# VUmcCGP/wisecondor

Hardware: NVIDIA B200
Metric: newref_bin_pairs_per_s (higher is better)
Workload: dtype f64

## Files before the change

wisecondor_b200/csrc/wc_common.cuh:

```cuda
#pragma once
#include <cuda.h>
#include <cuda_runtime.h>
#include <stdint.h>
#include <stdio.h>
#include <string.h>
#include <math.h>
#include <string>
#include <vector>
#include <algorithm>
#include "../../include/wisecondor_b200.h"

void wc_set_error(const char* fmt, ...);

#define WC_CUDA(expr)                                                                                   \
    do {                                                                                                \
        cudaError_t _e = (expr);                                                                        \
        if (_e != cudaSuccess) {                                                                        \
            wc_set_error("%s failed: %s (%s:%d)", #expr, cudaGetErrorString(_e), __FILE__, __LINE__);   \
            return WC_ERR_CUDA;                                                                         \
        }                                                                                               \
    } while (0)

#define WC_CHECK_ARG(cond)                                                                              \
    do {                                                                                                \
// ... 7 lines not shown
    void* p = nullptr;
    size_t bytes = 0;
};

enum { WC_NBUF = 56, WC_NPHASE = 12, WC_NCOUNTER = 12 };

enum {
    SLOT_XC = 0, SLOT_NORMS, SLOT_ROWCS, SLOT_ROWCE, SLOT_RBMETA, SLOT_CAND_D, SLOT_CAND_J, SLOT_SEGCNT,
    SLOT_SEGFLAG, SLOT_SLOW, SLOT_SCRATCH, SLOT_IO_X, SLOT_IO_IDX, SLOT_IO_DIST, SLOT_ROWTHR,
    SLOT_IN_KEY, SLOT_IN_J, SLOT_IN_CNT, SLOT_N32, SLOT_F16STAT,
    SLOT_PROF = 20, SLOT_PIV_IDS = 21, SLOT_PIV_X = 22, SLOT_PIV_N = 23, SLOT_PIV_META = 37, SLOT_S_STACK = 38,
    SLOT_T_COPY = 24, SLOT_T_ZT, SLOT_T_RT, SLOT_T_NT, SLOT_T_SD, SLOT_T_FLAGS, SLOT_T_TOTALS, SLOT_T_PROJ,
    SLOT_T_REVCNT = 44, SLOT_T_REVCUR, SLOT_T_DIRTY, SLOT_T_PAIRS,
    SLOT_S_ZC = 32, SLOT_S_META, SLOT_S_STATUS, SLOT_S_RC, SLOT_S_AUX,
    SLOT_P_FIRST = 40,
    SLOT_FIN_J = 48, SLOT_FIN_D, SLOT_FIN_P, SLOT_FIN_GRP
};

struct wc_shard_plan {
    int valid = 0;
    int N = 0, S = 0, k = 0, cap = 0, in_cap = 0, world = 1, rank = 0;
    int nb = 0, bp = 0, b0 = 0, b1 = 0;
    int row0 = 0, row1 = 0, rows_per = 0;
    int nkc = 0, nd_last = 0, extra_h = 0, ld = 0, nstages = 0, nrb = 0, nseg = 0, gridA = 0, gridB = 0;
    size_t Npad = 0, smem = 0, nlistA = 0;
    long long tilesA = 0, tilesB = 0, tiles_plain = 0;
    double mcoef = 0.0, madd = 0.0;
    int f16 = 0, ldh = 0;
    int pivots = 0;
    const double* corrected = nullptr;
    const unsigned long long* thr = nullptr;
// ... 125 lines not shown
```

wisecondor_b200/csrc/wc_search.cu:

```cuda
#include "wc_common.cuh"
#include <cuda_fp16.h>

namespace {

typedef unsigned long long u64;

constexpr int BM = 128;
constexpr int BN = 128;
constexpr int BK = 16;
constexpr int CONSUMER_WARPS = 8;
constexpr int CONSUMER_THREADS = CONSUMER_WARPS * 32;
constexpr int WROWS = BM / CONSUMER_WARPS;
constexpr int PRODUCER_WARPS = 4;
constexpr int TOPK_THREADS = CONSUMER_THREADS + PRODUCER_WARPS * 32;
constexpr int TILE_BYTES = BM * BK * 8;
constexpr int STAGE_BYTES = 2 * TILE_BYTES;
constexpr int MAX_STAGES = 6;
constexpr int HIST_BINS = 256;
constexpr int FIN_THREADS = 128;
constexpr int FIN_CHUNK = 32;
constexpr int FIN_BUCKETS = 1024;
constexpr int FIN_ECAP = 1360;
constexpr int EXH_THREADS = 256;
constexpr int STG = 128;
// ... 92 lines not shown
}
__device__ __forceinline__ int bucket_of(double d, double mn, float scale) {
    int b = (int)((float)(d - mn) * scale);
    return b < 0 ? 0 : (b > HIST_BINS - 1 ? HIST_BINS - 1 : b);
}
__device__ __forceinline__ u64 key_of_tau(double tau) { return (u64)__double_as_longlong(-0.5 * tau); }
inline u64 host_key_of_tau(double tau) {
    const double v = -0.5 * tau;
    u64 bits;
    memcpy(&bits, &v, sizeof(bits));
    return bits;
}
__device__ __forceinline__ double dist_of_key(u64 key) { return -2.0 * __longlong_as_double((long long)key); }
template <typename Args>
__device__ __forceinline__ double madd_of(const Args& a) { return a.madd_p != nullptr ? __ldg(a.madd_p) : a.madd; }

template <int PER_LANE>
__device__ __noinline__ void prune_row(u64* ck, int* cj, int n, int k, double nrm, double mcoef, double madd, int lane,
                                       u64* sk, int* sj, u64* thr_out, int* n_out) {
    (void)sk; (void)sj;
    u64 d[PER_LANE];
    int j[PER_LANE];
#pragma unroll
    for (int t = 0; t < PER_LANE; ++t) {
        const int i = t * 32 + lane;
        d[t] = i < n ? __ldcg(ck + i) : ~0ull;
        j[t] = i < n ? __ldcg(cj + i) : 0;
    }
    u64 lo = ~0ull, hi = 0ull;
#pragma unroll
// ... 477 lines not shown
    int k;
    int shortcap;
    double mcoef;
    int* idx_out;
    double* dist_out;
    int* slow_list;
    int* slow_count;
    int slow_bias;
    int vec;
    const u64* in_key;
    const int* in_j;
    const int* in_cnt;
    int in_cap;
    double madd;
    const double* madd_p;
    const u64* row_thr;
    int in_nsrc;
    int in_src_rows;
    int* sl_j;
    u64* sl_k;
    int* sl_p;
    int* grp;
    int* grp_count;
    const int* row_list;
    const int* row_count;
    int* stats;
    int* sl_b;
    int* bkt_hist;
    int bkt_shift;
};

template <int FT, bool SPLIT>
__device__ __forceinline__ void finalize_row(const FinArgs& a, const int rloc, unsigned char* fin_raw) {
    constexpr int ecap = FIN_ECAP;
    double* ex_d = reinterpret_cast<double*>(fin_raw + (size_t)ecap * 12);
    int* ex_j = reinterpret_cast<int*>(ex_d + a.shortcap);
    int* hist = ex_j + a.shortcap;
    __shared__ double s_red[2][FT / 32];
    __shared__ int s_total, s_flag, s_p, s_bstar, s_valid;

    const int tid = threadIdx.x, lane = tid & 31, warp = tid >> 5;
    const int row = a.row_begin + rloc;
    const int rb = rloc / BM, rl = rloc % BM;
    const int seg0 = a.rb_seg_first[rb], nseg = a.rb_seg_count[rb];
    int* out_i = a.idx_out + (size_t)rloc * a.k;
// ... 790 lines not shown
            if (sym)
                WC_CUDA(cudaMemcpyAsync(d_sym, sym_tab.data(), sym_tab.size() * sizeof(int), cudaMemcpyHostToDevice, stream));
            ctx->sched_hash = h;
        }
    }
    WC_CUDA(cudaMemsetAsync(slow, 0, sizeof(int), stream));
    WC_CUDA(cudaMemsetAsync(seg_cnt, 0, (size_t)std::max(nseg, 1) * BM * sizeof(int), stream));
    WC_CUDA(cudaMemsetAsync(seg_flag, 0, (size_t)std::max(nseg, 1) * BM * sizeof(int), stream));
    if (sym) WC_CUDA(cudaMemsetAsync(in_cnt, 0, (size_t)rows * sizeof(int), stream));

    bool f16 = ctx->k5_f16 != 0;
    const bool tc = ctx->k5_f16 == 2;
    const int ldh = tc ? (S + 4 + BKH - 1) / BKH * BKH : (S + BKH - 1) / BKH * BKH;
    const int ldx = tc ? ldh + BKH : ldh;
    float* n32 = nullptr;
    double nmax = 0.0;
    const double eps16 = ldexp(1.0, -10) * (1.0 + ldexp(1.0, -11)) + (tc ? 2.0 : 1.0) * (double)ldh * ldexp(1.0, -23) +
                         (tc ? ldexp(1.0, -20) : ldexp(1.0, -21));
    const unsigned long long* f16_stats_d = nullptr;
    WC_CUDA(cudaEventRecord(ctx->ev[0], stream));
    if (f16) {
        unsigned long long* stats;
        if ((rc = wc_reserve(ctx, SLOT_N32, Npad * sizeof(float), (void**)&n32))) return rc;
        if ((rc = wc_reserve(ctx, SLOT_F16STAT, 4 * sizeof(unsigned long long), (void**)&stats))) return rc;
        WC_CUDA(cudaMemsetAsync(stats, 0, 2 * sizeof(unsigned long long), stream));
        wc_prepare_f16_kernel<<<(int)((Npad * 32 + 255) / 256), 256, 0, stream>>>(corrected_d, N, (int)Npad, S, ldh, ldx, tc ? 1 : 0,
                                                                                  reinterpret_cast<__half*>(Xc), norms, n32, stats);
        WC_CUDA(cudaGetLastError());
        if (ctx->k5_f16_checked != 0) {
            f16_stats_d = stats;
            wc_f16_margin_kernel<<<1, 1, 0, stream>>>(stats, S, eps16, reinterpret_cast<double*>(stats + 2));
        } else {
            unsigned long long st_h[2] = {0, 0};
            WC_CUDA(cudaMemcpyAsync(st_h, stats, sizeof(st_h), cudaMemcpyDeviceToHost, stream));
            WC_CUDA(cudaStreamSynchronize(stream));
            memcpy(&nmax, &st_h[0], sizeof(double));
            if (st_h[1] != 0) f16 = false;
        }
    }
    if (!f16) {
        const int blocks = (int)((Npad * 32 + 255) / 256);
        wc_prepare_kernel<<<blocks, 256, 0, stream>>>(corrected_d, N, (int)Npad, S, ld, Sx, Xc, norms);
// ... 113 lines not shown
        ta.cta_piece_begin = d_cta_piece + (gridA + 1);
        launch(true, gridB);
    }
    WC_CUDA(cudaGetLastError());
    WC_CUDA(cudaEventRecord(ctx->ev[3], stream));

    FinArgs fa;
    fa.X = corrected_d; fa.N = N; fa.S = S; fa.norms = norms; fa.row_cs = d_row_cs; fa.row_ce = d_row_ce;
    fa.row_begin = row_begin; fa.row_end = row_end; fa.rb_seg_first = d_seg_first; fa.rb_seg_count = d_seg_count;
    fa.cand_key = cand_key; fa.cand_j = cand_j; fa.seg_cnt = seg_cnt; fa.seg_flag = seg_flag; fa.cap = cap; fa.k = k;
    fa.shortcap = k <= (f16 ? 96 : 128) ? 256 : 512;
    fa.mcoef = filt_mcoef; fa.idx_out = idx_d; fa.dist_out = dist_d; fa.slow_list = slow + 1; fa.slow_count = slow;
    fa.vec = (S % 4 == 0 && (reinterpret_cast<uintptr_t>(corrected_d) & 31) == 0) ? 4 : 1;
    fa.in_key = in_key; fa.in_j = in_j; fa.in_cnt = in_cnt; fa.in_cap = in_cap; fa.in_nsrc = 1; fa.in_src_rows = 0;
    fa.madd = filt_madd; fa.row_thr = row_thr; fa.madd_p = ta.madd_p;
    fa.slow_bias = 0;
    WC_CUDA(cudaEventRecord(ctx->ev[4], stream));
    long long fin_launches = 0;
    const int nparts = (ctx->d2h_idx_h != nullptr && rows >= 16 * BM) ? std::max(1, ctx->k6_parts) : 1;
    ctx->d2h_rows_done = 0;
    for (int pi = 0, r0 = 0; pi < nparts; ++pi) {
        const int r1 = pi + 1 == nparts ? (int)rows : (int)((long long)rows * (pi + 1) / nparts) / BM * BM;
        if (r1 <= r0) continue;
        FinArgs f = fa;
        const int hb = r0 / BM;
        f.row_begin = row_begin + r0; f.row_end = row_begin + r1;
        f.rb_seg_first += hb; f.rb_seg_count += hb;
        f.idx_out += (size_t)r0 * k; f.dist_out += (size_t)r0 * k;
        f.slow_bias = r0;
        if (f.row_thr != nullptr) f.row_thr += r0;
// ... 175 lines not shown
```

wisecondor_b200/csrc/wc_search_f16.cuh:

```cuda
#pragma once

constexpr int BKH = 64;
constexpr int F16_SCRATCH = 4096;

__device__ __forceinline__ void ldsm_x4(uint32_t addr, uint32_t& r0, uint32_t& r1, uint32_t& r2, uint32_t& r3) {
    asm volatile("ldmatrix.sync.aligned.m8n8.x4.shared.b16 {%0,%1,%2,%3}, [%4];"
                 : "=r"(r0), "=r"(r1), "=r"(r2), "=r"(r3) : "r"(addr));
}
__device__ __forceinline__ void hmma_16816(float (&c)[4], uint32_t a0, uint32_t a1, uint32_t a2, uint32_t a3, uint32_t b0,
                                           uint32_t b1) {
    asm volatile("mma.sync.aligned.m16n8k16.row.col.f32.f16.f16.f32 {%0,%1,%2,%3}, {%4,%5,%6,%7}, {%8,%9}, {%0,%1,%2,%3};"
                 : "+f"(c[0]), "+f"(c[1]), "+f"(c[2]), "+f"(c[3]) : "r"(a0), "r"(a1), "r"(a2), "r"(a3), "r"(b0), "r"(b1));
}
__device__ __forceinline__ float tau32_of_key(u64 key) { return __double2float_ru(dist_of_key(key)); }

__global__ void wc_prepare_f16_kernel(const double* __restrict__ X, int N, int Npad, int S, int ldh, int ldx, int fold,
                                      __half* __restrict__ Xh, double* __restrict__ norms, float* __restrict__ n32,
                                      unsigned long long* __restrict__ stats) {
    const int row = (int)(((size_t)blockIdx.x * blockDim.x + threadIdx.x) >> 5);
    const int lane = threadIdx.x & 31;
    if (row >= Npad) return;
    __half* dst = Xh + (size_t)row * ldx;
    double acc = 0.0;
    bool big = false;
    if (row < N) {
        const double* src = X + (size_t)row * S;
        for (int s = lane; s < ldh; s += 32) {
            const double v = s < S ? src[s] - 1.0 : 0.0;
            const __half hv = __double2half(v);
            dst[s] = hv;
            if (fold && s >= ldh - BKH) dst[s + BKH] = hv;
            acc = fma(v, v, acc);
            if (fabs(v) > 60000.0 && fabs(v) < INFINITY) big = true;
        }
    } else {
        for (int s = lane; s < ldx; s += 32) dst[s] = __float2half(0.0f);
    }
#pragma unroll
    for (int o = 16; o > 0; o >>= 1) acc += __shfl_xor_sync(0xffffffffu, acc, o);
    big = __any_sync(0xffffffffu, big);
    __syncwarp();
    if (lane == 0) {
        norms[row] = row < N ? acc : 0.0;
        n32[row] = row < N ? (float)acc : INFINITY;
        if (fold && row < N) {
            const double nh = -0.5 * acc;
            if (!(acc * 0.5 <= 60000.0)) big = true;
            const __half h = __double2half(nh);
            const __half l = __double2half(nh - (double)__half2float(h));
            const __half one = __float2half(1.0f);
            dst[ldh - 4] = h;   dst[ldh - 3] = l;   dst[ldh - 2] = one; dst[ldh - 1] = one;
            dst[ldx - 4] = one; dst[ldx - 3] = one; dst[ldx - 2] = h;   dst[ldx - 1] = l;
        }
        if (row < N && acc < INFINITY) atomicMax(stats, (unsigned long long)__double_as_longlong(acc));
        if (big) atomicOr(stats + 1, 1ull);
    }
}

template <bool SYM>
// ... 348 lines not shown
```

wisecondor_b200/csrc/wc_search_fin.cuh:

```cuda
#pragma once

constexpr int SEL_WARPS = 4;
constexpr int SEL_ECAP = 1024;
constexpr int SEL_EPL = SEL_ECAP / 32;
constexpr int SEL_U = 4;
constexpr int SEL_MAXSRC = 255;
constexpr size_t SEL_WARP_BYTES = (size_t)SEL_ECAP * 12 + (SEL_MAXSRC + 1) * 4 + 12;
constexpr size_t SEL_WARP_STRIDE = (SEL_WARP_BYTES + 15) / 16 * 16;

__global__ void __launch_bounds__(SEL_WARPS * 32) wc_fin_select_kernel(const FinArgs a, int* __restrict__ big_list,
                                                                       int* __restrict__ big_count, int* __restrict__ stats) {
    extern __shared__ __align__(16) unsigned char sel_raw[];
    const int lane = threadIdx.x & 31, warp = threadIdx.x >> 5;
    const int rloc = blockIdx.x * SEL_WARPS + warp;
    const int rows = a.row_end - a.row_begin;
    if (rloc >= rows) return;
    u64* en_k = reinterpret_cast<u64*>(sel_raw + (size_t)warp * SEL_WARP_STRIDE);
    int* en_j = reinterpret_cast<int*>(en_k + SEL_ECAP);
    int* pre = en_j + SEL_ECAP;
    const int row = a.row_begin + rloc;
    const int rb = rloc / BM, rl = rloc % BM;
    const int seg0 = a.rb_seg_first[rb], nseg = a.rb_seg_count[rb];
    const int nsrc = nseg + (a.in_key != nullptr ? a.in_nsrc : 0);
    int* out_i = a.idx_out + (size_t)rloc * a.k;
// ... 78 lines not shown
            if (keep && pos < SEL_ECAP) {
                en_k[pos] = key[u];
                en_j[pos] = jj[u];
            }
            kept += __popc(bm);
        }
    }
    if (kept > SEL_ECAP) { to_big(); return; }
    if (kept == 0) {
        for (int e = lane; e < a.k; e += 32) { out_i[e] = -1; out_d[e] = 1e10; }
        if (lane == 0) a.sl_p[rloc] = -1;
        return;
    }
    __syncwarp();
    u64 d[SEL_EPL];
#pragma unroll
    for (int t = 0; t < SEL_EPL; ++t) d[t] = t * 32 + lane < kept ? en_k[t * 32 + lane] : ~0ull;
    u64 lo = ~0ull, hi = 0ull;
#pragma unroll
    for (int t = 0; t < SEL_EPL; ++t) {
        if (t * 32 + lane < kept) {
            lo = d[t] < lo ? d[t] : lo;
            hi = d[t] > hi ? d[t] : hi;
        }
    }
    lo = warp_min_u64(lo);
    hi = warp_max_u64(hi);
    u64 blo = lo, bhi = hi, cut = hi;
    int c_hi = kept;
    for (int it = 0; it < 70 && c_hi > a.k; ++it) {
        if (bhi - blo < 2) break;
        const u64 mid = blo + ((bhi - blo) >> 1);
// ... 1 lines not shown
#pragma unroll
        for (int t = 0; t < SEL_EPL; ++t) c += d[t] <= mid ? 1 : 0;
#pragma unroll
        for (int o = 16; o > 0; o >>= 1) c += __shfl_xor_sync(0xffffffffu, c, o);
        if (c >= a.k) { bhi = mid; c_hi = c; cut = mid; } else { blo = mid; }
    }
    u64 vstar = 0ull;
#pragma unroll
    for (int t = 0; t < SEL_EPL; ++t)
        if (d[t] <= cut && d[t] > vstar) vstar = d[t];
    vstar = warp_max_u64(vstar);
    const double dv = dist_of_key(vstar);
    double window = fmax(dv, 0.0) + a.mcoef * (a.norms[row] + fabs(dv)) + madd_of(a);
    if (!(window > 1e-300)) window = 1e-300;
    const u64 wkey = key_of_tau(window);
    int p = 0, jmin = 0x7fffffff;
#pragma unroll
    for (int t = 0; t < SEL_EPL; ++t) {
        const bool keep = t * 32 + lane < kept && d[t] <= wkey;
        const unsigned bm = __ballot_sync(0xffffffffu, keep);
        const int pos = p + __popc(bm & ((1u << lane) - 1u));
        if (keep && pos < a.shortcap) {
            const int j = en_j[t * 32 + lane];
            a.sl_j[(size_t)rloc * a.shortcap + pos] = j;
            jmin = min(jmin, j);
        }
        p += __popc(bm);
    }
#pragma unroll
    for (int o = 16; o > 0; o >>= 1) jmin = min(jmin, __shfl_xor_sync(0xffffffffu, jmin, o));
    if (lane == 0) {
        if (p > a.shortcap) {
            a.slow_list[atomicAdd(a.slow_count, 1)] = rloc + a.slow_bias;
            a.sl_p[rloc] = -1;
        } else {
            a.sl_p[rloc] = p;
            const int bkt = min(jmin >> a.bkt_shift, FIN_BUCKETS - 1);
            a.sl_b[rloc] = bkt;
            atomicAdd(a.bkt_hist + bkt, (p + 31) >> 5);
            if (stats != nullptr) { atomicAdd(stats, kept); atomicAdd(stats + 1, p); atomicMax(stats + 2, kept); }
        }
    }
}

constexpr int SELH_WARPS = 8;
constexpr int SELH_BINS = 1024;

__global__ void __launch_bounds__(SELH_WARPS * 32, 5) wc_fin_select_hist_kernel(const FinArgs a, int* __restrict__ big_list,
                                                                            int* __restrict__ big_count, int* __restrict__ stats) {
    __shared__ int s_hist[SELH_WARPS][SELH_BINS];
    __shared__ int s_pre[SELH_WARPS][SEL_MAXSRC + 1];
    const int lane = threadIdx.x & 31, warp = threadIdx.x >> 5;
    const int rloc = blockIdx.x * SELH_WARPS + warp;
    const int rows = a.row_end - a.row_begin;
    if (rloc >= rows) return;
    int* hist = s_hist[warp];
    int* pre = s_pre[warp];
    const int row = a.row_begin + rloc;
    const int rb = rloc / BM, rl = rloc % BM;
    const int seg0 = a.rb_seg_first[rb], nseg = a.rb_seg_count[rb];
    const int nsrc = nseg + (a.in_key != nullptr ? a.in_nsrc : 0);
    int* out_i = a.idx_out + (size_t)rloc * a.k;
// ... 27 lines not shown
        if (s0 == 0 && lane == 0) pre[0] = 0;
        __syncwarp();
    }
    if (__any_sync(0xffffffffu, flagged != 0)) {
        if (lane == 0) { a.slow_list[atomicAdd(a.slow_count, 1)] = rloc + a.slow_bias; a.sl_p[rloc] = -1; }
        return;
    }
    const u64 tfinal = a.row_thr != nullptr ? __ldcg(a.row_thr + rloc) : ~0ull;
    auto sweep = [&](auto&& f) {
        int s = 0, e0 = 0, ns = nsrc > 0 ? pre[1] : 0;
        bool more = true;
        while (more) {
            u64 key[SEL_U];
            int jj[SEL_U];
            bool ok[SEL_U];
#pragma unroll
            for (int u = 0; u < SEL_U; ++u) {
                while (s < nsrc && e0 >= ns) { ++s; e0 = 0; ns = s < nsrc ? pre[s + 1] - pre[s] : 0; }
                key[u] = ~0ull;
                jj[u] = 0;
                ok[u] = false;
                if (s < nsrc) {
                    const int e = e0 + lane;
                    if (e < ns) {
                        ok[u] = true;
                        if (s < nseg) {
                            const size_t off = ((size_t)(seg0 + s) * BM + rl) * a.cap + e;
                            key[u] = a.cand_key[off];
                            jj[u] = a.cand_j[off];
                        } else {
                            const size_t off = ((size_t)(s - nseg) * a.in_src_rows + rloc) * a.in_cap + e;
                            key[u] = a.in_key[off];
                            jj[u] = a.in_j[off];
                        }
                    }
                    e0 += 32;
                } else {
                    more = false;
                }
            }
#pragma unroll
            for (int u = 0; u < SEL_U; ++u) f(key[u], jj[u], ok[u]);
        }
    };
    double d0 = 0.0, dmax = dist_of_key(tfinal);
    if (!(dmax < 1e10)) {
        const double cut = 1e10 + a.mcoef * (a.norms[row] + 1e10) + madd_of(a);
        double mn = INFINITY, mx = -INFINITY;
        sweep([&](u64 key, int, bool valid) {
            const double d = dist_of_key(key);
            if (valid && key <= tfinal && d <= cut) { mn = fmin(mn, d); mx = fmax(mx, d); }
        });
#pragma unroll
        for (int o = 16; o > 0; o >>= 1) {
            mn = fmin(mn, __shfl_xor_sync(0xffffffffu, mn, o));
            mx = fmax(mx, __shfl_xor_sync(0xffffffffu, mx, o));
        }
        if (mx >= mn) { d0 = mn; dmax = mx; } else { dmax = 0.0; }
    }
    const float scale = dmax - d0 > 1e-5 * fabs(dmax) ? (float)SELH_BINS / (float)(dmax - d0) : 0.0f;
    auto bucket = [&](double d) -> int {
        const float x = (float)(d - d0) * scale;
        return x < (float)SELH_BINS ? (x >= 0.0f ? (int)x : 0) : SELH_BINS - 1;
    };
    int kept = 0;
    sweep([&](u64 key, int, bool valid) {
        const bool live = valid && key <= tfinal;
        if (live) atomicAdd(&hist[bucket(dist_of_key(key))], 1);
        kept += __popc(__ballot_sync(0xffffffffu, live));
    });
    if (kept == 0) {
        for (int e = lane; e < a.k; e += 32) { out_i[e] = -1; out_d[e] = 1e10; }
        if (lane == 0) a.sl_p[rloc] = -1;
        return;
    }
    __syncwarp();
    auto kth_bucket = [&](int kk, int& below) -> int {
        constexpr int PER = SELH_BINS / 32;
        static_assert(PER % 32 == 0, "one bank per lane in the rotated read");
        int sum = 0;
#pragma unroll 8
        for (int t = 0; t < PER; ++t) sum += hist[lane * PER + ((t + lane) & (PER - 1))];
        int incl = sum;
// ... 16 lines not shown
                if (lane >= o) inc2 += w;
            }
            const unsigned m2 = __ballot_sync(0xffffffffu, base + inc2 >= kk);
            if (m2) {
                const int l2 = __ffs(m2) - 1;
                below = base + __shfl_sync(0xffffffffu, inc2 - v, l2);
                return lstar * PER + r * 32 + l2;
            }
            base += __shfl_sync(0xffffffffu, inc2, 31);
        }
        return -1;
    };
    int below = 0;
    int bstar = kth_bucket(a.k, below);
    const bool refine = bstar >= 0 && bstar < SELH_BINS - 1 && scale > 0.0f;
    double vstar = dmax;
    if (refine) vstar = fmin(dmax, d0 + (double)(__fdividef((float)(bstar + 1), scale) * (1.0f + 8.0f * 1.1920929e-7f)));
    auto window_key = [&](double v) -> u64 {
        double window = fmax(v, 0.0) + a.mcoef * (a.norms[row] + fabs(v)) + madd_of(a);
        if (!(window > 1e-300)) window = 1e-300;
        const u64 wk = key_of_tau(window);
        return wk > tfinal ? tfinal : wk;
    };
    const u64 wkey = window_key(vstar);
    const int edge_cnt = refine ? hist[bucket(dist_of_key(wkey))] : 0;
    __syncwarp();
    for (int bb = lane; bb < SELH_BINS; bb += 32) hist[bb] = 0;
    __syncwarp();
    const double dscale = (double)scale;
    u64* my_k = a.sl_k + (size_t)rloc * a.shortcap;
    int* my_j = a.sl_j + (size_t)rloc * a.shortcap;
    int p = 0, jmin = 0x7fffffff;
    sweep([&](u64 key, int j, bool valid) {
        const bool keep = valid && key <= wkey;
        const unsigned bm = __ballot_sync(0xffffffffu, keep);
        const int pos = p + __popc(bm & ((1u << lane) - 1u));
        if (keep && pos < a.shortcap) {
            my_j[pos] = j;
            my_k[pos] = key;
            jmin = min(jmin, j);
        }
        p += __popc(bm);
        if (refine && keep) {
            const double d = dist_of_key(key);
            if (bucket(d) == bstar) {
                const double f = ((d - d0) * dscale - (double)bstar) * (double)SELH_BINS;
                atomicAdd(&hist[f < (double)SELH_BINS ? (f >= 0.0 ? (int)f : 0) : SELH_BINS - 1], 1);
            }
        }
    });
    if (p > a.shortcap) {
        if (lane == 0) {
            a.slow_list[atomicAdd(a.slow_count, 1)] = rloc + a.slow_bias;
            a.sl_p[rloc] = -1;
        }
        return;
    }
    __syncwarp();
    if (refine && p > a.k && ((p - 1) >> 5) != ((max(a.k, p - 2 * edge_cnt - 2) - 1) >> 5)) {
        int below2 = 0;
        const int sstar = kth_bucket(a.k - below, below2);
        if (sstar >= 0 && sstar < SELH_BINS - 1) {
            const double v2 = d0 + ((double)bstar + ((double)(sstar + 1) + 1e-3) / (double)SELH_BINS) / dscale;
            const u64 wkey2 = window_key(fmin(vstar, v2));
            if (wkey2 < wkey) {
                int q = 0;
                jmin = 0x7fffffff;
                for (int e0 = 0; e0 < p; e0 += 32) {
                    const int e = e0 + lane;
                    const bool keep = e < p && __ldcg(my_k + e) <= wkey2;
                    const int j = e < p ? __ldcg(my_j + e) : 0;
                    __syncwarp();
                    const unsigned bm = __ballot_sync(0xffffffffu, keep);
                    if (keep) {
                        my_j[q + __popc(bm & ((1u << lane) - 1u))] = j;
                        jmin = min(jmin, j);
                    }
                    q += __popc(bm);
                }
                p = q;
            }
        }
    }
#pragma unroll
    for (int o = 16; o > 0; o >>= 1) jmin = min(jmin, __shfl_xor_sync(0xffffffffu, jmin, o));
// ... 350 lines not shown
    fa.sl_k = reinterpret_cast<u64*>(sl_d);
    if ((rc = wc_reserve(ctx, SLOT_FIN_P, (2 * (size_t)rows + 8 + FIN_BUCKETS) * sizeof(int), (void**)&fa.sl_p))) return rc;
    if ((rc = wc_reserve(ctx, SLOT_FIN_GRP, (size_t)rows * (gpr + 1) * sizeof(int), (void**)&fa.grp))) return rc;
    fa.grp_count = fa.sl_p + rows;
    int* big_count = fa.sl_p + rows + 1;
    int* stats = fa.sl_p + rows + 2;
    fa.sl_b = fa.sl_p + rows + 8;
    fa.bkt_hist = fa.sl_b + rows;
    fa.bkt_shift = 0;
    while (((fa.N - 1) >> fa.bkt_shift) >= FIN_BUCKETS) ++fa.bkt_shift;
    WC_CUDA(cudaMemsetAsync(fa.bkt_hist, 0, FIN_BUCKETS * sizeof(int), stream));
    int* big_list = fa.grp + (size_t)rows * gpr;
    WC_CUDA(cudaMemsetAsync(fa.grp_count, 0, 5 * sizeof(int), stream));
    fa.row_list = nullptr; fa.row_count = nullptr; fa.stats = stats;
    if (ctx->k6_select != 0) {
        wc_fin_select_hist_kernel<<<(rows + SELH_WARPS - 1) / SELH_WARPS, SELH_WARPS * 32, 0, stream>>>(fa, big_list, big_count, stats);
    } else {
        const size_t sel_smem = SEL_WARPS * SEL_WARP_STRIDE;
        WC_CUDA(cudaFuncSetAttribute(wc_fin_select_kernel, cudaFuncAttributeMaxDynamicSharedMemorySize, (int)sel_smem));
        wc_fin_select_kernel<<<(rows + SEL_WARPS - 1) / SEL_WARPS, SEL_WARPS * 32, sel_smem, stream>>>(fa, big_list, big_count, stats);
    }
    WC_CUDA(cudaGetLastError());
    {
        fa.row_list = big_list; fa.row_count = big_count;
        const int g = std::min(rows, 8 * ctx->sm_count);
        if (wide) {
            WC_CUDA(cudaFuncSetAttribute(wc_finalize_kernel<160, true>, cudaFuncAttributeMaxDynamicSharedMemorySize, (int)fin_smem));
            wc_finalize_kernel<160, true><<<g, 160, fin_smem, stream>>>(fa);
        } else {
            WC_CUDA(cudaFuncSetAttribute(wc_finalize_kernel<FIN_THREADS, true>, cudaFuncAttributeMaxDynamicSharedMemorySize, (int)fin_smem));
            wc_finalize_kernel<FIN_THREADS, true><<<g, FIN_THREADS, fin_smem, stream>>>(fa);
        }
        WC_CUDA(cudaGetLastError());
    }
    wc_fin_bucket_scan_kernel<<<1, FIN_BUCKETS, 0, stream>>>(fa.bkt_hist, fa.grp_count);
// ... 76 lines not shown
```

wisecondor_b200/csrc/wc_search_shard.cuh:

```cuda
#pragma once

namespace {

struct ShardDims { int nb, bp, b0, b1, row0, row1, rows_per, in_cap, frac; size_t thr_len; };

ShardDims shard_dims(const wc_ctx* ctx, int N, int k, int world, int rank) {
    ShardDims d;
    d.frac = (ctx != nullptr && ctx->k5_sym >= 2) ? ctx->k5_sym : 8;
    d.nb = (N + BM - 1) / BM;
    d.bp = (d.nb + world - 1) / world;
    d.b0 = std::min(d.nb, rank * d.bp);
    d.b1 = std::min(d.nb, d.b0 + d.bp);
    d.row0 = std::min(N, d.b0 * BM);
    d.row1 = std::min(N, d.b1 * BM);
    d.rows_per = d.bp * BM;
    d.thr_len = (size_t)world * d.rows_per + BN;
    const int want = world == 1 ? 2 * k * d.frac : (4 * k * d.frac + world - 1) / world;
    d.in_cap = 256;
    while (d.in_cap < want) d.in_cap *= 2;
    return d;
}

int shard_launch_pass(wc_ctx* ctx, int pass, unsigned long long* thr_d, unsigned long long* in_key_d, int* in_j_d,
                      int* in_cnt_d, cudaStream_t stream, const std::vector<int>* seg_first = nullptr, int pivots = 0) {
// ... 207 lines not shown
    if ((rc = wc_reserve(ctx, SLOT_SEGFLAG, (size_t)std::max(nseg, 1) * BM * sizeof(int), (void**)&seg_flag))) return rc;
    const int rows = d.row1 - d.row0;
    if ((rc = wc_reserve(ctx, SLOT_SLOW, ((size_t)std::max(rows, 0) + 1) * sizeof(int), (void**)&slow))) return rc;
    WC_CUDA(cudaMemcpyAsync(d_row_cs, row_cs.data(), (size_t)N * sizeof(int), cudaMemcpyHostToDevice, stream));
    WC_CUDA(cudaMemcpyAsync(d_row_ce, row_ce.data(), (size_t)N * sizeof(int), cudaMemcpyHostToDevice, stream));
    WC_CUDA(cudaMemcpyAsync(d_meta, meta.data(), meta.size() * sizeof(int), cudaMemcpyHostToDevice, stream));
    WC_CUDA(cudaMemsetAsync(slow, 0, sizeof(int), stream));
    WC_CUDA(cudaMemsetAsync(seg_cnt, 0, (size_t)std::max(nseg, 1) * BM * sizeof(int), stream));
    WC_CUDA(cudaMemsetAsync(seg_flag, 0, (size_t)std::max(nseg, 1) * BM * sizeof(int), stream));

    bool f16 = ctx->k5_f16 != 0;
    const bool tcf = ctx->k5_f16 == 2;
    const int ldh = tcf ? (S + 4 + BKH - 1) / BKH * BKH : (S + BKH - 1) / BKH * BKH;
    const int ldx = tcf ? ldh + BKH : ldh;
    double nmax = 0.0;
    WC_CUDA(cudaEventRecord(ctx->ev[0], stream));
    if (f16) {
        float* n32;
        unsigned long long* stats;
        if ((rc = wc_reserve(ctx, SLOT_N32, Npad * sizeof(float), (void**)&n32))) return rc;
        if ((rc = wc_reserve(ctx, SLOT_F16STAT, 2 * sizeof(unsigned long long), (void**)&stats))) return rc;
        WC_CUDA(cudaMemsetAsync(stats, 0, 2 * sizeof(unsigned long long), stream));
        wc_prepare_f16_kernel<<<(int)((Npad * 32 + 255) / 256), 256, 0, stream>>>(corrected_d, N, (int)Npad, S, ldh, ldx, tcf ? 1 : 0,
                                                                                  reinterpret_cast<__half*>(Xc), norms, n32, stats);
        WC_CUDA(cudaGetLastError());
        unsigned long long st_h[2] = {0, 0};
        WC_CUDA(cudaMemcpyAsync(st_h, stats, sizeof(st_h), cudaMemcpyDeviceToHost, stream));
        WC_CUDA(cudaStreamSynchronize(stream));
        memcpy(&nmax, &st_h[0], sizeof(double));
        if (st_h[1] != 0) f16 = false;
    }
    if (!f16)
        wc_prepare_kernel<<<(int)((Npad * 32 + 255) / 256), 256, 0, stream>>>(corrected_d, N, (int)Npad, S, ld, Sx, Xc, norms);
    WC_CUDA(cudaGetLastError());
    WC_CUDA(cudaEventRecord(ctx->ev[1], stream));
    const double eps16 = ldexp(1.0, -10) * (1.0 + ldexp(1.0, -11)) + (tcf ? 2.0 : 1.0) * (double)ldh * ldexp(1.0, -23) +
                         (tcf ? ldexp(1.0, -20) : ldexp(1.0, -21));
    const double tau_init = f16 ? 3e38 : 1e10 * (1.0 + 1e-6);
    wc_fill_u64_kernel<<<(unsigned)((N + 255) / 256), 256, 0, stream>>>(thr_d, (size_t)N, host_key_of_tau(tau_init));
    wc_fill_u64_kernel<<<(unsigned)((d.thr_len - N + 255) / 256), 256, 0, stream>>>(thr_d + N, d.thr_len - (size_t)N, KEY_NEVER);
    WC_CUDA(cudaGetLastError());

    pl.N = N; pl.S = S; pl.k = k; pl.cap = cap; pl.in_cap = d.in_cap; pl.world = world; pl.rank = rank;
    pl.nb = nb; pl.bp = d.bp; pl.b0 = d.b0; pl.b1 = d.b1; pl.row0 = d.row0; pl.row1 = d.row1; pl.rows_per = d.rows_per;
    pl.nkc = nkc; pl.nd_last = nd_last; pl.extra_h = nd_last; pl.ld = ld; pl.nrb = nrb; pl.nseg = npieces;
    pl.gridA = gridA; pl.gridB = gridB; pl.Npad = Npad; pl.nlistA = listA.size();
    pl.tilesA = tilesA; pl.tilesB = tilesB; pl.tiles_plain = tiles_plain;
    pl.f16 = f16 ? ctx->k5_f16 : 0;
    pl.ldh = ldh;
    pl.mcoef = f16 ? 2.0 * eps16 : 16.0 * (double)(S + 16) * 1.1102230246251565e-16;
    pl.madd = f16 ? 2.0 * eps16 * nmax + ldexp(1.0, -20) * sqrt((double)S * nmax) : 0.0;
    if (f16) pl.nkc = ldh / BKH;
// ... 59 lines not shown
    if (rows > 0) {
        WC_CHECK_ARG(idx_d != nullptr && dist_d != nullptr);
        const int nrb1 = std::max(pl.nrb, 1);
        FinArgs fa;
        fa.X = pl.corrected; fa.N = pl.N; fa.S = pl.S; fa.norms = static_cast<double*>(ctx->buf[SLOT_NORMS].p);
        fa.row_cs = d_row_cs; fa.row_ce = d_row_ce; fa.row_begin = pl.row0; fa.row_end = pl.row1;
        fa.rb_seg_first = d_meta + 2 * nrb1; fa.rb_seg_count = d_meta + 3 * nrb1;
        fa.cand_key = static_cast<u64*>(ctx->buf[SLOT_CAND_D].p); fa.cand_j = static_cast<int*>(ctx->buf[SLOT_CAND_J].p);
        fa.seg_cnt = static_cast<int*>(ctx->buf[SLOT_SEGCNT].p); fa.seg_flag = static_cast<int*>(ctx->buf[SLOT_SEGFLAG].p);
        fa.cap = pl.cap; fa.k = pl.k; fa.shortcap = pl.k <= (pl.f16 ? 96 : 128) ? 256 : 512; fa.mcoef = pl.mcoef;
        fa.idx_out = idx_d; fa.dist_out = dist_d; fa.slow_list = slow + 1; fa.slow_count = slow; fa.slow_bias = 0;
        fa.vec = (pl.S % 4 == 0 && (reinterpret_cast<uintptr_t>(pl.corrected) & 31) == 0) ? 4 : 1;
        fa.in_key = recv_key_d; fa.in_j = recv_j_d; fa.in_cnt = recv_cnt_d; fa.in_cap = pl.in_cap;
        fa.in_nsrc = pl.world; fa.in_src_rows = pl.rows_per; fa.madd = pl.madd; fa.madd_p = nullptr;
        fa.row_thr = pl.thr != nullptr ? pl.thr + pl.row0 : nullptr;
        WC_CUDA(cudaEventRecord(ctx->ev[4], stream));
        long long fin_launches = 0;
        int rcf;
        if ((rcf = launch_finalize(ctx, stream, fa, rows, pl.f16 != 0, &fin_launches))) return rcf;
        launches += fin_launches - 1;
        WC_CUDA(cudaEventRecord(ctx->ev[5], stream));
        int k6_stats[4] = {0, 0, 0, 0};
        WC_CUDA(cudaMemcpyAsync(&nslow, slow, sizeof(int), cudaMemcpyDeviceToHost, stream));
        if (ctx->k6_stats_d != nullptr) WC_CUDA(cudaMemcpyAsync(k6_stats, ctx->k6_stats_d, 4 * sizeof(int), cudaMemcpyDeviceToHost, stream));
        WC_CUDA(cudaStreamSynchronize(stream));
        ctx->counter[8] = k6_stats[1];
        ctx->counter[9] = k6_stats[2];
    ctx->counter[10] = k6_stats[0];
    ctx->counter[11] = k6_stats[3];
        if (nslow > 0) {
// ... 35 lines not shown
```

Measured before the change: 481.7 billion.

## Use per-pair error bounds for candidate pruning in f16 finalize select

Computes a per-row error weight (from eps and norm) in the f16 prepare kernel and stores it in a new buffer. The finalize select kernels, templated on a PP flag, use interval bounds (d ± wi+wj) per candidate pair instead of a single row-wide window. The aim is fewer survivors passed to exact f64 refinement. This adds a gather of pw[j] per candidate and extra arithmetic, and changes the selection logic, which risks correctness if the bounds are wrong.

```diff
diff --git a/wisecondor_b200/csrc/wc_common.cuh b/wisecondor_b200/csrc/wc_common.cuh
--- a/wisecondor_b200/csrc/wc_common.cuh
+++ b/wisecondor_b200/csrc/wc_common.cuh
@@ -45,7 +45,8 @@
     SLOT_T_REVCNT = 44, SLOT_T_REVCUR, SLOT_T_DIRTY, SLOT_T_PAIRS,
     SLOT_S_ZC = 32, SLOT_S_META, SLOT_S_STATUS, SLOT_S_RC, SLOT_S_AUX,
     SLOT_P_FIRST = 40,
-    SLOT_FIN_J = 48, SLOT_FIN_D, SLOT_FIN_P, SLOT_FIN_GRP
+    SLOT_FIN_J = 48, SLOT_FIN_D, SLOT_FIN_P, SLOT_FIN_GRP,
+    SLOT_PAIRW = 52
 };
 
 struct wc_shard_plan {
diff --git a/wisecondor_b200/csrc/wc_search.cu b/wisecondor_b200/csrc/wc_search.cu
--- a/wisecondor_b200/csrc/wc_search.cu
+++ b/wisecondor_b200/csrc/wc_search.cu
@@ -130,6 +130,13 @@
 __device__ __forceinline__ double dist_of_key(u64 key) { return -2.0 * __longlong_as_double((long long)key); }
 template <typename Args>
 __device__ __forceinline__ double madd_of(const Args& a) { return a.madd_p != nullptr ? __ldg(a.madd_p) : a.madd; }
+
+__device__ __forceinline__ void pair_bounds(double d, double wi, double wj, double& lo, double& hi) {
+    const double e = __dadd_ru(wi, wj);
+    lo = __dadd_rd(d, -e);
+    hi = __dadd_ru(d, e);
+}
+
 
 template <int PER_LANE>
 __device__ __noinline__ void prune_row(u64* ck, int* cj, int n, int k, double nrm, double mcoef, double madd, int lane,
@@ -637,6 +644,7 @@
     int in_cap;
     double madd;
     const double* madd_p;
+    const double* pw;
     const u64* row_thr;
     int in_nsrc;
     int in_src_rows;
@@ -652,6 +660,7 @@
     int* bkt_hist;
     int bkt_shift;
 };
+
 
 template <int FT, bool SPLIT>
 __device__ __forceinline__ void finalize_row(const FinArgs& a, const int rloc, unsigned char* fin_raw) {
@@ -1472,6 +1481,7 @@
     const int ldh = tc ? (S + 4 + BKH - 1) / BKH * BKH : (S + BKH - 1) / BKH * BKH;
     const int ldx = tc ? ldh + BKH : ldh;
     float* n32 = nullptr;
+    double* pw = nullptr;
     double nmax = 0.0;
     const double eps16 = ldexp(1.0, -10) * (1.0 + ldexp(1.0, -11)) + (tc ? 2.0 : 1.0) * (double)ldh * ldexp(1.0, -23) +
                          (tc ? ldexp(1.0, -20) : ldexp(1.0, -21));
@@ -1480,10 +1490,12 @@
     if (f16) {
         unsigned long long* stats;
         if ((rc = wc_reserve(ctx, SLOT_N32, Npad * sizeof(float), (void**)&n32))) return rc;
+        if ((rc = wc_reserve(ctx, SLOT_PAIRW, (size_t)N * sizeof(double), (void**)&pw))) return rc;
         if ((rc = wc_reserve(ctx, SLOT_F16STAT, 4 * sizeof(unsigned long long), (void**)&stats))) return rc;
         WC_CUDA(cudaMemsetAsync(stats, 0, 2 * sizeof(unsigned long long), stream));
         wc_prepare_f16_kernel<<<(int)((Npad * 32 + 255) / 256), 256, 0, stream>>>(corrected_d, N, (int)Npad, S, ldh, ldx, tc ? 1 : 0,
-                                                                                  reinterpret_cast<__half*>(Xc), norms, n32, stats);
+                                                                                  reinterpret_cast<__half*>(Xc), norms, n32, stats,
+                                                                                  eps16, pw);
         WC_CUDA(cudaGetLastError());
         if (ctx->k5_f16_checked != 0) {
             f16_stats_d = stats;
@@ -1627,6 +1639,7 @@
     fa.vec = (S % 4 == 0 && (reinterpret_cast<uintptr_t>(corrected_d) & 31) == 0) ? 4 : 1;
     fa.in_key = in_key; fa.in_j = in_j; fa.in_cnt = in_cnt; fa.in_cap = in_cap; fa.in_nsrc = 1; fa.in_src_rows = 0;
     fa.madd = filt_madd; fa.row_thr = row_thr; fa.madd_p = ta.madd_p;
+    fa.pw = f16 ? pw : nullptr;
     fa.slow_bias = 0;
     WC_CUDA(cudaEventRecord(ctx->ev[4], stream));
     long long fin_launches = 0;
diff --git a/wisecondor_b200/csrc/wc_search_f16.cuh b/wisecondor_b200/csrc/wc_search_f16.cuh
--- a/wisecondor_b200/csrc/wc_search_f16.cuh
+++ b/wisecondor_b200/csrc/wc_search_f16.cuh
@@ -16,7 +16,7 @@
 
 __global__ void wc_prepare_f16_kernel(const double* __restrict__ X, int N, int Npad, int S, int ldh, int ldx, int fold,
                                       __half* __restrict__ Xh, double* __restrict__ norms, float* __restrict__ n32,
-                                      unsigned long long* __restrict__ stats) {
+                                      unsigned long long* __restrict__ stats, double eps, double* __restrict__ pw) {
     const int row = (int)(((size_t)blockIdx.x * blockDim.x + threadIdx.x) >> 5);
     const int lane = threadIdx.x & 31;
     if (row >= Npad) return;
@@ -43,6 +43,7 @@
     if (lane == 0) {
         norms[row] = row < N ? acc : 0.0;
         n32[row] = row < N ? (float)acc : INFINITY;
+        if (row < N) pw[row] = __fma_ru(eps, acc, __dmul_ru(ldexp(1.0, -22), __dsqrt_ru(__dmul_ru((double)S, acc))));
         if (fold && row < N) {
             const double nh = -0.5 * acc;
             if (!(acc * 0.5 <= 60000.0)) big = true;
diff --git a/wisecondor_b200/csrc/wc_search_fin.cuh b/wisecondor_b200/csrc/wc_search_fin.cuh
--- a/wisecondor_b200/csrc/wc_search_fin.cuh
+++ b/wisecondor_b200/csrc/wc_search_fin.cuh
@@ -8,6 +8,7 @@
 constexpr size_t SEL_WARP_BYTES = (size_t)SEL_ECAP * 12 + (SEL_MAXSRC + 1) * 4 + 12;
 constexpr size_t SEL_WARP_STRIDE = (SEL_WARP_BYTES + 15) / 16 * 16;
 
+template <bool PP>
 __global__ void __launch_bounds__(SEL_WARPS * 32) wc_fin_select_kernel(const FinArgs a, int* __restrict__ big_list,
                                                                        int* __restrict__ big_count, int* __restrict__ stats) {
     extern __shared__ __align__(16) unsigned char sel_raw[];
@@ -116,8 +117,18 @@
     }
     __syncwarp();
     u64 d[SEL_EPL];
-#pragma unroll
-    for (int t = 0; t < SEL_EPL; ++t) d[t] = t * 32 + lane < kept ? en_k[t * 32 + lane] : ~0ull;
+    const double wi = PP ? a.pw[row] : 0.0;
+    auto bounds = [&](int e, double& lo, double& hi) { pair_bounds(dist_of_key(en_k[e]), wi, __ldg(a.pw + en_j[e]), lo, hi); };
+#pragma unroll
+    for (int t = 0; t < SEL_EPL; ++t) {
+        const int e = t * 32 + lane;
+        d[t] = e < kept ? en_k[e] : ~0ull;
+        if (PP && e < kept) {
+            double lo, hi;
+            bounds(e, lo, hi);
+            d[t] = hi == hi ? key_of_tau(hi) : ~0ull;
+        }
+    }
     u64 lo = ~0ull, hi = 0ull;
 #pragma unroll
     for (int t = 0; t < SEL_EPL; ++t) {
@@ -149,10 +160,16 @@
     double window = fmax(dv, 0.0) + a.mcoef * (a.norms[row] + fabs(dv)) + madd_of(a);
     if (!(window > 1e-300)) window = 1e-300;
     const u64 wkey = key_of_tau(window);
+    const double bound_lo = vstar == ~0ull ? 1e10 : fmin(fmax(dv, 0.0), 1e10);
     int p = 0, jmin = 0x7fffffff;
 #pragma unroll
     for (int t = 0; t < SEL_EPL; ++t) {
-        const bool keep = t * 32 + lane < kept && d[t] <= wkey;
+        bool keep = t * 32 + lane < kept && d[t] <= wkey;
+        if (PP) {
+            double lo = 0.0, hi;
+            if (t * 32 + lane < kept) bounds(t * 32 + lane, lo, hi);
+            keep = t * 32 + lane < kept && lo <= bound_lo;
+        }
         const unsigned bm = __ballot_sync(0xffffffffu, keep);
         const int pos = p + __popc(bm & ((1u << lane) - 1u));
         if (keep && pos < a.shortcap) {
@@ -181,6 +198,7 @@
 constexpr int SELH_WARPS = 8;
 constexpr int SELH_BINS = 1024;
 
+template <bool PP>
 __global__ void __launch_bounds__(SELH_WARPS * 32, 5) wc_fin_select_hist_kernel(const FinArgs a, int* __restrict__ big_list,
                                                                             int* __restrict__ big_count, int* __restrict__ stats) {
     __shared__ int s_hist[SELH_WARPS][SELH_BINS];
@@ -238,6 +256,7 @@
             u64 key[SEL_U];
             int jj[SEL_U];
             bool ok[SEL_U];
+            double wj[SEL_U];
 #pragma unroll
             for (int u = 0; u < SEL_U; ++u) {
                 while (s < nsrc && e0 >= ns) { ++s; e0 = 0; ns = s < nsrc ? pre[s + 1] - pre[s] : 0; }
@@ -264,16 +283,26 @@
                 }
             }
 #pragma unroll
-            for (int u = 0; u < SEL_U; ++u) f(key[u], jj[u], ok[u]);
+            for (int u = 0; u < SEL_U; ++u) wj[u] = PP && ok[u] ? __ldg(a.pw + jj[u]) : 0.0;
+#pragma unroll
+            for (int u = 0; u < SEL_U; ++u) f(key[u], jj[u], wj[u], ok[u]);
         }
     };
+    const double wi = PP ? a.pw[row] : 0.0;
+    auto bounds = [&](u64 key, double wj, double& lo, double& hi) { pair_bounds(dist_of_key(key), wi, wj, lo, hi); };
     double d0 = 0.0, dmax = dist_of_key(tfinal);
     if (!(dmax < 1e10)) {
-        const double cut = 1e10 + a.mcoef * (a.norms[row] + 1e10) + madd_of(a);
+        const double cut = PP ? 0.0 : 1e10 + a.mcoef * (a.norms[row] + 1e10) + madd_of(a);
         double mn = INFINITY, mx = -INFINITY;
-        sweep([&](u64 key, int, bool valid) {
-            const double d = dist_of_key(key);
-            if (valid && key <= tfinal && d <= cut) { mn = fmin(mn, d); mx = fmax(mx, d); }
+        sweep([&](u64 key, int, double wj, bool valid) {
+            double d = dist_of_key(key);
+            bool in = d <= cut;
+            if (PP) {
+                double lo;
+                bounds(key, wj, lo, d);
+                in = lo <= 1e10;
+            }
+            if (valid && key <= tfinal && in) { mn = fmin(mn, d); mx = fmax(mx, d); }
         });
 #pragma unroll
         for (int o = 16; o > 0; o >>= 1) {
@@ -288,9 +317,16 @@
         return x < (float)SELH_BINS ? (x >= 0.0f ? (int)x : 0) : SELH_BINS - 1;
     };
     int kept = 0;
-    sweep([&](u64 key, int, bool valid) {
+    double hmax = -INFINITY;
+    sweep([&](u64 key, int, double wj, bool valid) {
         const bool live = valid && key <= tfinal;
-        if (live) atomicAdd(&hist[bucket(dist_of_key(key))], 1);
+        double d = dist_of_key(key);
+        if (PP) {
+            double lo;
+            bounds(key, wj, lo, d);
+            if (live) hmax = fmax(hmax, d);
+        }
+        if (live) atomicAdd(&hist[bucket(d)], 1);
         kept += __popc(__ballot_sync(0xffffffffu, live));
     });
     if (kept == 0) {
@@ -337,16 +373,24 @@
     int below = 0;
     int bstar = kth_bucket(a.k, below);
     const bool refine = bstar >= 0 && bstar < SELH_BINS - 1 && scale > 0.0f;
-    double vstar = dmax;
+    if (PP) {
+#pragma unroll
+        for (int o = 16; o > 0; o >>= 1) hmax = fmax(hmax, __shfl_xor_sync(0xffffffffu, hmax, o));
+    }
+    double vstar = PP ? hmax : dmax;
     if (refine) vstar = fmin(dmax, d0 + (double)(__fdividef((float)(bstar + 1), scale) * (1.0f + 8.0f * 1.1920929e-7f)));
+    auto lo_bound = [&](double v) -> double { return fmin(v, 1e10); };
+    const double bstar_lo = lo_bound(vstar);
     auto window_key = [&](double v) -> u64 {
         double window = fmax(v, 0.0) + a.mcoef * (a.norms[row] + fabs(v)) + madd_of(a);
         if (!(window > 1e-300)) window = 1e-300;
         const u64 wk = key_of_tau(window);
         return wk > tfinal ? tfinal : wk;
     };
-    const u64 wkey = window_key(vstar);
-    const int edge_cnt = refine ? hist[bucket(dist_of_key(wkey))] : 0;
+    const u64 wkey = PP ? tfinal : window_key(vstar);
+    double edge = dist_of_key(wkey);
+    if (PP) edge = vstar + 4.0 * wi;
+    const int edge_cnt = refine ? hist[bucket(edge)] : 0;
     __syncwarp();
     for (int bb = lane; bb < SELH_BINS; bb += 32) hist[bb] = 0;
     __syncwarp();
@@ -354,18 +398,25 @@
     u64* my_k = a.sl_k + (size_t)rloc * a.shortcap;
     int* my_j = a.sl_j + (size_t)rloc * a.shortcap;
     int p = 0, jmin = 0x7fffffff;
-    sweep([&](u64 key, int j, bool valid) {
-        const bool keep = valid && key <= wkey;
+    sweep([&](u64 key, int j, double wj, bool valid) {
+        bool keep = valid && key <= wkey;
+        double d = dist_of_key(key);
+        u64 park = key;
+        if (PP) {
+            double lo;
+            bounds(key, wj, lo, d);
+            keep = keep && lo <= bstar_lo;
+            park = (u64)__double_as_longlong(lo);
+        }
         const unsigned bm = __ballot_sync(0xffffffffu, keep);
         const int pos = p + __popc(bm & ((1u << lane) - 1u));
         if (keep && pos < a.shortcap) {
             my_j[pos] = j;
-            my_k[pos] = key;
+            my_k[pos] = park;
             jmin = min(jmin, j);
         }
         p += __popc(bm);
         if (refine && keep) {
-            const double d = dist_of_key(key);
             if (bucket(d) == bstar) {
                 const double f = ((d - d0) * dscale - (double)bstar) * (double)SELH_BINS;
                 atomicAdd(&hist[f < (double)SELH_BINS ? (f >= 0.0 ? (int)f : 0) : SELH_BINS - 1], 1);
@@ -385,13 +436,15 @@
         const int sstar = kth_bucket(a.k - below, below2);
         if (sstar >= 0 && sstar < SELH_BINS - 1) {
             const double v2 = d0 + ((double)bstar + ((double)(sstar + 1) + 1e-3) / (double)SELH_BINS) / dscale;
-            const u64 wkey2 = window_key(fmin(vstar, v2));
-            if (wkey2 < wkey) {
+            const u64 wkey2 = PP ? 0ull : window_key(fmin(vstar, v2));
+            const double lo2 = PP ? lo_bound(fmin(vstar, v2)) : 0.0;
+            if (PP ? lo2 < bstar_lo : wkey2 < wkey) {
                 int q = 0;
                 jmin = 0x7fffffff;
                 for (int e0 = 0; e0 < p; e0 += 32) {
                     const int e = e0 + lane;
-                    const bool keep = e < p && __ldcg(my_k + e) <= wkey2;
+                    const u64 pk = e < p ? __ldcg(my_k + e) : 0ull;
+                    const bool keep = e < p && (PP ? __longlong_as_double((long long)pk) <= lo2 : pk <= wkey2);
                     const int j = e < p ? __ldcg(my_j + e) : 0;
                     __syncwarp();
                     const unsigned bm = __ballot_sync(0xffffffffu, keep);
@@ -772,11 +825,13 @@
     WC_CUDA(cudaMemsetAsync(fa.grp_count, 0, 5 * sizeof(int), stream));
     fa.row_list = nullptr; fa.row_count = nullptr; fa.stats = stats;
     if (ctx->k6_select != 0) {
-        wc_fin_select_hist_kernel<<<(rows + SELH_WARPS - 1) / SELH_WARPS, SELH_WARPS * 32, 0, stream>>>(fa, big_list, big_count, stats);
+        auto kern = fa.pw != nullptr ? wc_fin_select_hist_kernel<true> : wc_fin_select_hist_kernel<false>;
+        kern<<<(rows + SELH_WARPS - 1) / SELH_WARPS, SELH_WARPS * 32, 0, stream>>>(fa, big_list, big_count, stats);
     } else {
         const size_t sel_smem = SEL_WARPS * SEL_WARP_STRIDE;
-        WC_CUDA(cudaFuncSetAttribute(wc_fin_select_kernel, cudaFuncAttributeMaxDynamicSharedMemorySize, (int)sel_smem));
-        wc_fin_select_kernel<<<(rows + SEL_WARPS - 1) / SEL_WARPS, SEL_WARPS * 32, sel_smem, stream>>>(fa, big_list, big_count, stats);
+        auto kern = fa.pw != nullptr ? wc_fin_select_kernel<true> : wc_fin_select_kernel<false>;
+        WC_CUDA(cudaFuncSetAttribute(kern, cudaFuncAttributeMaxDynamicSharedMemorySize, (int)sel_smem));
+        kern<<<(rows + SEL_WARPS - 1) / SEL_WARPS, SEL_WARPS * 32, sel_smem, stream>>>(fa, big_list, big_count, stats);
     }
     WC_CUDA(cudaGetLastError());
     {
diff --git a/wisecondor_b200/csrc/wc_search_shard.cuh b/wisecondor_b200/csrc/wc_search_shard.cuh
--- a/wisecondor_b200/csrc/wc_search_shard.cuh
+++ b/wisecondor_b200/csrc/wc_search_shard.cuh
@@ -245,15 +245,20 @@
     const int ldh = tcf ? (S + 4 + BKH - 1) / BKH * BKH : (S + BKH - 1) / BKH * BKH;
     const int ldx = tcf ? ldh + BKH : ldh;
     double nmax = 0.0;
+    const double eps16 = ldexp(1.0, -10) * (1.0 + ldexp(1.0, -11)) + (tcf ? 2.0 : 1.0) * (double)ldh * ldexp(1.0, -23) +
+                         (tcf ? ldexp(1.0, -20) : ldexp(1.0, -21));
     WC_CUDA(cudaEventRecord(ctx->ev[0], stream));
     if (f16) {
         float* n32;
+        double* pw;
         unsigned long long* stats;
         if ((rc = wc_reserve(ctx, SLOT_N32, Npad * sizeof(float), (void**)&n32))) return rc;
+        if ((rc = wc_reserve(ctx, SLOT_PAIRW, (size_t)N * sizeof(double), (void**)&pw))) return rc;
         if ((rc = wc_reserve(ctx, SLOT_F16STAT, 2 * sizeof(unsigned long long), (void**)&stats))) return rc;
         WC_CUDA(cudaMemsetAsync(stats, 0, 2 * sizeof(unsigned long long), stream));
         wc_prepare_f16_kernel<<<(int)((Npad * 32 + 255) / 256), 256, 0, stream>>>(corrected_d, N, (int)Npad, S, ldh, ldx, tcf ? 1 : 0,
-                                                                                  reinterpret_cast<__half*>(Xc), norms, n32, stats);
+                                                                                  reinterpret_cast<__half*>(Xc), norms, n32, stats,
+                                                                                  eps16, pw);
         WC_CUDA(cudaGetLastError());
         unsigned long long st_h[2] = {0, 0};
         WC_CUDA(cudaMemcpyAsync(st_h, stats, sizeof(st_h), cudaMemcpyDeviceToHost, stream));
@@ -265,8 +270,6 @@
         wc_prepare_kernel<<<(int)((Npad * 32 + 255) / 256), 256, 0, stream>>>(corrected_d, N, (int)Npad, S, ld, Sx, Xc, norms);
     WC_CUDA(cudaGetLastError());
     WC_CUDA(cudaEventRecord(ctx->ev[1], stream));
-    const double eps16 = ldexp(1.0, -10) * (1.0 + ldexp(1.0, -11)) + (tcf ? 2.0 : 1.0) * (double)ldh * ldexp(1.0, -23) +
-                         (tcf ? ldexp(1.0, -20) : ldexp(1.0, -21));
     const double tau_init = f16 ? 3e38 : 1e10 * (1.0 + 1e-6);
     wc_fill_u64_kernel<<<(unsigned)((N + 255) / 256), 256, 0, stream>>>(thr_d, (size_t)N, host_key_of_tau(tau_init));
     wc_fill_u64_kernel<<<(unsigned)((d.thr_len - N + 255) / 256), 256, 0, stream>>>(thr_d + N, d.thr_len - (size_t)N, KEY_NEVER);
@@ -356,6 +359,7 @@
         fa.in_key = recv_key_d; fa.in_j = recv_j_d; fa.in_cnt = recv_cnt_d; fa.in_cap = pl.in_cap;
         fa.in_nsrc = pl.world; fa.in_src_rows = pl.rows_per; fa.madd = pl.madd; fa.madd_p = nullptr;
         fa.row_thr = pl.thr != nullptr ? pl.thr + pl.row0 : nullptr;
+        fa.pw = pl.f16 ? static_cast<const double*>(ctx->buf[SLOT_PAIRW].p) : nullptr;
         WC_CUDA(cudaEventRecord(ctx->ev[4], stream));
         long long fin_launches = 0;
         int rcf;
```

New measurement: 469.9 billion (median of 6 runs). -2.5%, worse.
